# NREL/sup3r

Measured on AMD Instinct MI355X. Metric: samples/sec (lo-res chunks), generator forward, 5x/12x ST-GAN, higher is better.
Workload: dtype bf16

## Files before the change

### sup3r_amd/csrc/common.h

```cpp
#pragma once
#include <hip/hip_runtime.h>
#include <stdint.h>

#include <atomic>
#include <mutex>
#include <string>
#include <vector>

#include "../../include/sup3r_hip.h"
#include "launch_shape.h"


#define S3_OPTION_LIST(X) \
  X(BF16_TRAIN_ACT) \
  X(DENSE_WGS) \
  X(DGRAD_S2_MIN_TILES) \
  X(DISC_BF16) \
  X(FEWCH_HALO_MIN_TILES) \
  X(FP32_ACT) \
  X(GCONV_MF2) \
  X(GCONV_MF4) \
  X(GRAPH) \
  X(HALO32_MIN_TILES) \
  X(HALO_S2_MIN_TILES) \
  X(MFMA_DBG) \
  X(MFMA_TILE) \
  X(NO_BATCHED_PACK) \
  X(NO_BIAS_FUSE) \
  X(NO_CHUNKED_DY16) \
  X(NO_DGRAD_C2) \
  X(NO_DGRAD_C2_SLIDE) \
  X(DGRAD_C2_SLIDE_MIN_UNITS) \
  X(NO_DGRAD_CHUNKED) \
  X(NO_DGRAD_FEWCH) \
  X(NO_DGRAD_S2) \
  X(NO_DGRAD_X3) \
  X(NO_DIRECT_OUTPUT) \
  X(NO_DISC_BF16) \
  X(NO_DPRE16) \
  X(NO_DPRE16_ONLY_MASK) \
  X(NO_FEWCH) \
  X(NO_FEWCH_HALO) \
  X(NO_FEWPOS) \
  X(NO_FEWPOS_MFMA) \
  X(NO_FEWPOS_BWD_FUSE) \
  X(NO_FEWPOS_SMALL) \
  X(NO_FEWPOS_TRUNK) \
  X(NO_FOLD16) \
  X(NO_FRAME16) \
  X(NO_FUSED2D) \
  X(NO_GCONV) \
  X(NO_GCONV_DY16) \
  X(NO_GCONV_SPLITK) \
  X(NO_HALO32) \
  X(NO_HALO_S2) \
  X(NO_MASK_FUSE) \
  X(NO_MFMA_GEN) \
  X(NO_DGRAD_GEN) \
  X(NO_CONV2D_WS) \
  X(NO_TRAIN2D_BF16) \
  X(NO_ADD16) \
  X(NO_WS_EXO) \
  X(NO_WS_RES2) \
  X(NO_WS_PP) \
  X(NO_WS_X3) \
  X(WS_X3_MIN_POS) \
  X(NO_CONV2D_OUT) \
  X(NO_CONV2D_HEAD) \
  X(KEEP_ACTIVATIONS) \
  X(NO_MFMA_BWD) \
  X(NO_PERSIST) \
  X(NO_PERSIST_DGRAD) \
  X(NO_PERSIST_STRIP) \
  X(PERSIST2) \
  X(NO_REPEAT_FUSE) \
  X(NO_WGRAD_X3) \
  X(NO_GCONV_X3) \
  X(NO_SIGN_BYTES) \
  X(NO_HALO_S2_K64) \
  X(NO_PLAIN_FOLD16) \
  X(NO_SEG_REDUCE) \
  X(NO_TAIL_BAND) \
  X(NO_TAIL_MFMA) \
  X(NO_TAIL_SLIDE) \
  X(NO_TAIL_SWEEP) \
  X(NO_TAIL_WINDOW) \
  X(NO_TAIL_X3) \
  X(NO_TILE66) \
  X(NO_TILE_NF2) \
  X(NO_WGRAD_BF16) \
  X(NO_WGRAD_C2) \
  X(NO_WGRAD_GEN_PF) \
  X(NO_WGRAD_TAIL) \
  X(NO_WGRAD_TAIL_SWEEP) \
  X(NO_WGRAD_WS) \
  X(PERSIST_DGRAD_MIN_TILES) \
  X(PERSIST_MIN_TILES) \
  X(POISON_ALLOC) \
  X(TAIL_SWEEP_SHAPE) \
  X(TRACE) \
  X(WGRAD_DBG) \
  X(WGRAD_SIDE_STREAM)
enum S3OptId {
#define X(n) S3O_##n,
  S3_OPTION_LIST(X)
#undef X
  S3O_COUNT
};
struct S3Options {
  int32_t v[S3O_COUNT];
  bool has[S3O_COUNT];
  S3Options() { for (int i = 0; i < S3O_COUNT; ++i) { v[i] = 0; has[i] = false; } }
};
extern thread_local const S3Options* s3_active_options;
const char* s3_option_name(int id);
int s3_option_id(const char* name);
inline bool s3_opt_has(int id) { return s3_active_options && s3_active_options->has[id]; }
inline long long s3_opt_int(int id, long long dflt) { return s3_opt_has(id) ? s3_active_options->v[id] : dflt; }
inline bool s3_opt_on(int id) { return s3_opt_int(id, 0) != 0; }
struct S3OptScope {
  const S3Options* prev;
  explicit S3OptScope(const S3Options* o) : prev(s3_active_options) { s3_active_options = o; }
  ~S3OptScope() { s3_active_options = prev; }
};

struct s3_ctx {
// ... 28 lines not shown
  std::mutex m;
  bool done(int dev) const { return (mask.load(std::memory_order_acquire) >> (dev & 63)) & 1u; }
  void mark(int dev) { mask.fetch_or(1ull << (dev & 63), std::memory_order_release); }
};

#define S3_HIP(ctx, call)                                                    \
  do {                                                                       \
    hipError_t e_ = (call);                                                  \
    if (e_ != hipSuccess) {                                                  \
      (ctx)->err = std::string(#call) + ": " + hipGetErrorString(e_);        \
      return S3_EHIP;                                                        \
    }                                                                        \
  } while (0)

#define S3_FAIL(ctx, code, msg) \
  do {                          \
    (ctx)->err = (msg);         \
    return (code);              \
  } while (0)

inline int s3_lds_set(s3_ctx*) { return S3_OK; }
template <class K, class B, class... Rest>
int s3_lds_set(s3_ctx* ctx, K* kernel, B bytes, Rest... rest) {
  S3_HIP(ctx, hipFuncSetAttribute(reinterpret_cast<const void*>(kernel),
                                  hipFuncAttributeMaxDynamicSharedMemorySize, (int)bytes));
  return s3_lds_set(ctx, rest...);
}
template <class... Pairs>
inline int s3_lds_optin(s3_ctx* ctx, S3DeviceOnce& once, Pairs... pairs) {
  if (once.done(ctx->device)) return S3_OK;
  std::lock_guard<std::mutex> lk(once.m);
  const int rc = s3_lds_set(ctx, pairs...);
  if (rc == S3_OK) once.mark(ctx->device);
  return rc;
}

struct ConvGeom {
  int N;
  int D[3];
  int O[3];
  int Cin, Cout;
  int k[3], s[3], lo[3];
  int pad_mode;
  int act;
  float alpha;
  int d2s;
  int in_cstride = 0, in_cvalid = 0;
  int w_cin = 0;
  const float* exo = nullptr;
  const void* res2 = nullptr;
  int ws_only = 0;
  int in_rep = 0;
  int res_rep = 0;
  int gen = 0;
  int64_t xn = 0, yn = 0;
  int64_t xs[3] = {0, 0, 0}, ys[3] = {0, 0, 0}, yb[2] = {0, 0};
};

struct GatherGeom {
  int kind;
  int N;
  int Di[3], Ci;
  int Do[3], Co;
  int lo[3];
  int pad_mode;
  int rep;
  int d2s;
  int c_off;
};

__host__ __device__ inline int s3_reflect(int i, int n) {
  if (i < 0) i = -i;
  if (i > n - 1) i = 2 * (n - 1) - i;
  return i;
}

struct FastDiv {
  uint32_t d = 1, m = 1, sh1 = 0, sh2 = 0;
  FastDiv() = default;
  explicit FastDiv(uint32_t div) : d(div) {
    uint32_t l = 0;
    while (l < 32 && ((uint64_t)1 << l) < div) ++l;
    m = (uint32_t)((((uint64_t)1 << 32) * (((uint64_t)1 << l) - div)) / div + 1);
    sh1 = l < 1 ? l : 1;
    sh2 = l < 1 ? 0 : l - 1;
  }
  __device__ __forceinline__ uint32_t operator()(uint32_t x) const {
    const uint32_t t = __umulhi(m, x);
    return (t + ((x - t) >> sh1)) >> sh2;
  }
};

__device__ inline int s3_xcd_tile(int b, int nblk) {
  const int q = nblk / 8, r = nblk % 8, xcd = b % 8, k = b / 8;
  return (xcd < r ? xcd * (q + 1) : r * (q + 1) + (xcd - r) * q) + k;
}

__device__ inline void s3_xcd_share(int64_t n, int64_t& lo, int64_t& hi, int& k, int& nk) {
  const int G = gridDim.x, b = blockIdx.x, xcd = b % 8;
  int before = 0;
  for (int q = 0; q < xcd; ++q) before += (G - q + 7) / 8;
  nk = (G - xcd + 7) / 8;
  k = b / 8;
  lo = n * before / G;
  hi = n * (before + nk) / G;
}
// ... 298 lines not shown
```

### sup3r_amd/csrc/kernels_conv_mfma_persist.hip

```cpp
#include <cstdlib>

#include "wave_prims.h"

namespace {

constexpr int TS0 = 4, TS1 = 8, TS2 = 16;
constexpr int H0 = TS0 + 2, H1 = TS1 + 2, H2 = TS2 + 2;
constexpr int HP = H0 * H1 * H2;
constexpr int HALO_BYTES = HP * 128;
constexpr int SLAB_OFF = HALO_BYTES;
constexpr int BIAS_OFF = SLAB_OFF + 3 * 8192;
constexpr int LDS_BYTES = BIAS_OFF + 256;

constexpr int NCW = 8;
constexpr int NPW = 4;
constexpr int NTHR = (NCW + NPW) * 64;
constexpr int MFW = TS0 * TS1 / NCW;
constexpr int PT = NPW * 64;
constexpr int ROWC = H1 * H2;
constexpr int JR = (ROWC * 8 + PT - 1) / PT;
constexpr int NLATE = (H0 - 2) * JR;
static_assert(MFW * NCW == TS0 * TS1 && TS1 % MFW == 0 && MFW == 4, "tile / wave split");
static_assert(JR <= 6 && NLATE <= 24, "producer tap schedule");

constexpr int early_k(int t) { return (t >= 0 && t < JR) || (t >= 9 && t < 9 + JR) ? 1 : 0; }
constexpr int late_k(int t) { return t >= 0 && t < NLATE ? 1 : 0; }
constexpr int halo_k(int t) { return early_k(t) + late_k(t); }

template <int TW>
struct PGeo {
  static constexpr int TS1 = TW, H1 = TW + 2;
  static constexpr int HP = H0 * H1 * H2, HALO_BYTES = HP * 128, SLAB_OFF = HALO_BYTES;
  static constexpr int BIAS_OFF = SLAB_OFF + 3 * 8192, LDS_BYTES = BIAS_OFF + 256;
  static constexpr int MFW = TS0 * TW / NCW;
  static constexpr int ROWC = H1 * H2;
  static constexpr int JR = (ROWC * 8 + PT - 1) / PT;
  static constexpr int NLATE = (H0 - 2) * JR;
  static_assert(MFW * NCW == TS0 * TW && TW % MFW == 0 && (MFW == 4 || MFW == 3), "tile / wave split");
  static_assert(JR <= 6 && NLATE <= 24 && H0 + H1 + H2 <= 64, "producer tap schedule / halo table");
  static constexpr int early_k(int t) { return (t >= 0 && t < JR) || (t >= 9 && t < 9 + JR) ? 1 : 0; }
  static constexpr int late_k(int t) { return t >= 0 && t < NLATE ? 1 : 0; }
  static constexpr int halo_k(int t) { return early_k(t) + late_k(t); }
};

__device__ inline u32x4 ld16_async(const void* sbase, unsigned voff) {
  u32x4 v;
  asm volatile("global_load_dwordx4 %0, %1, %2" : "=v"(v) : "v"(voff), "s"(sbase) : "memory");
  return v;
}
__device__ inline void wait_vm_n(int n) {
  switch (n) {
    case 0: WAIT_VM(0); break;
    case 1: WAIT_VM(1); break;
    case 2: WAIT_VM(2); break;
    case 3: WAIT_VM(3); break;
    case 4: WAIT_VM(4); break;
    case 5: WAIT_VM(5); break;
    default: WAIT_VM(6); break;
  }
}

__global__ void pack_persist_kernel(const float* __restrict__ w,
                                    unsigned short* __restrict__ out, int cout, int n_ct) {
  const int total = n_ct * 27 * 64 * 64;
  for (int idx = blockIdx.x * blockDim.x + threadIdx.x; idx < total;
       idx += gridDim.x * blockDim.x) {
    const int ci = idx & 63, rho = (idx >> 6) & 63, tap = (idx >> 12) % 27, ct = (idx >> 12) / 27;
    const int co = ct * 64 + slab_row_cout(rho);
    const float v = co < cout ? w[((size_t)tap * 64 + ci) * cout + co] : 0.f;
    const unsigned u = pk2(v, 0.f);
    const int slot = (ci >> 3) ^ ((rho >> 1) & 7);
    out[(((size_t)ct * 27 + tap) * 64 + rho) * 64 + slot * 8 + (ci & 7)] = (unsigned short)(u & 0xFFFFu);
  }
}

__global__ void pack_jobs_kernel(const S3PackJob* __restrict__ jobs) {
  const S3PackJob jb = jobs[blockIdx.y];
  const int total = jb.n_ct * 27 * 64 * 64;
  for (int idx = blockIdx.x * blockDim.x + threadIdx.x; idx < total; idx += gridDim.x * blockDim.x) {
    const int ci = idx & 63, row = (idx >> 6) & 63, tap = (idx >> 12) % 27, ct = (idx >> 12) / 27;
    const int co = ct * 64 + row;
    float v = 0.f;
    if (co < jb.cout)
      v = jb.dgrad ? jb.w[((size_t)(26 - tap) * jb.cout + co) * 64 + ci]
                   : jb.w[((size_t)tap * 64 + ci) * jb.cout + co];
    const unsigned short h = (unsigned short)(pk2(v, 0.f) & 0xFFFFu);
    const size_t base = (((size_t)ct * 27 + tap) * 64) * 64;
    const int sw = (ci >> 3);
    jb.tile[base + (size_t)row * 64 + ((sw ^ ((row >> 1) & 7)) << 3) + (ci & 7)] = h;
    if (jb.persist) {
      const int nf = ((row >> 5) << 1) | ((row >> 2) & 1), kq = (row >> 3) & 3, r = row & 3;
      const int rho = nf * 16 + kq * 4 + r;
      jb.persist[base + (size_t)rho * 64 + ((sw ^ ((rho >> 1) & 7)) << 3) + (ci & 7)] = h;
    }
  }
}

template <int NFV, bool DG, int REP = 0, bool RIN = false, bool F16 = false, int TW = 8>
__global__ __launch_bounds__(NTHR) void conv3_mfma_persist_kernel(
    const unsigned short* __restrict__ x, const char* __restrict__ wimg,
    const float* __restrict__ bias, const unsigned short* __restrict__ res,
    unsigned short* __restrict__ y, ConvGeom g, int tiles0, int tiles1,
    int tiles2, int n_tiles, int ct, int gs0, int gs1) {
  using PG = PGeo<TW>;
  constexpr int TS1 = PG::TS1, H1 = PG::H1, HP = PG::HP, SLAB_OFF = PG::SLAB_OFF, BIAS_OFF = PG::BIAS_OFF;
  constexpr int MFW = PG::MFW, ROWC = PG::ROWC, JR = PG::JR, NLATE = PG::NLATE;
  (void)HP;
  extern __shared__ __attribute__((aligned(16))) char smem[];
  const int tid = threadIdx.x;
  const int lane = tid & 63;
  const int wave = __builtin_amdgcn_readfirstlane(tid >> 6);
  const int D0 = g.D[0], D1 = g.D[1], D2 = g.D[2];

  int h_cur, h_end;
  {
    const int nblk = gridDim.x, b = blockIdx.x;
    const int xcd = b % 8, k = b / 8;
    int rank = k;
    for (int xx = 0; xx < xcd; ++xx) rank += (nblk - xx + 7) / 8;
    const long long H = n_tiles;
    h_cur = (int)((rank * H) / nblk);
    h_end = (int)(((rank + 1) * H) / nblk);
  }
  auto tile_org = [&](int h, int& n, int& o0, int& o1, int& o2) __attribute__((always_inline)) {
    int tr = h;
    o0 = (tr % tiles0) * 2; tr /= tiles0;
    o2 = (tr % tiles2) * TS2; tr /= tiles2;
    o1 = (tr % tiles1) * TS1 + (DG ? 0 : gs1); tr /= tiles1;
    n = tr;
  };
  auto item_at = [&](int h, int& hs0, int& nr) __attribute__((always_inline)) {
    const bool whole = hs0 + 1 < tiles0 && h + 1 < h_end;
    nr = whole ? 4 : 2;
    hs0 += whole ? 2 : 1;
    if (hs0 >= tiles0) hs0 = 0;
    return h + (whole ? 2 : 1);
  };

  if (wave >= NCW) {
    const int pt = tid - NCW * 64;
    const int pw = wave - NCW;
    const unsigned dma_voff = (unsigned)(pw * 2048 + lane * 16);
    auto dma_slab = [&](int tap, int slot) __attribute__((always_inline)) {
      unsigned vo;
      asm volatile("v_mov_b32 %0, %1" : "=v"(vo) : "v"(dma_voff));
      const char* sb = wimg + (size_t)tap * 8192 + vo;
      char* d = smem + SLAB_OFF + slot * 8192 + __builtin_amdgcn_readfirstlane((int)vo);
      __builtin_amdgcn_global_load_lds(
          (const __attribute__((address_space(1))) void*)sb,
          (__attribute__((address_space(3))) void*)d, 16, 0, 0);
      __builtin_amdgcn_global_load_lds(
          (const __attribute__((address_space(1))) void*)(sb + 1024),
          (__attribute__((address_space(3))) void*)(d + 1024), 16, 0, 0);
    };
    const int pcell = pt >> 3, pch = pt & 7;
    const bool cdead = DG && g.in_cstride && pch * 8 >= g.in_cvalid;
    u32x4 hlate[NLATE], hrow[JR];
    unsigned in_off[JR];
    unsigned lds_off[JR];
    int htab = 0;
    const unsigned short* hx = x;
#pragma unroll
    for (int j = 0; j < JR; ++j) {
      int cell = pcell + 32 * j;
      if (cell > ROWC - 1) cell = ROWC - 1;
      lds_off[j] = (unsigned)(cell * 128 + ((pch ^ ((cell % H2) & 7)) << 4));
    }
#define HALO_TABLE(tile_expr)                                                          \
    {                                                                                  \
      int n_, o0_, o1_, o2_;                                                           \
      tile_org((tile_expr), n_, o0_, o1_, o2_);                                        \
      n_ = __builtin_amdgcn_readfirstlane(n_);                                         \
      const int ax = lane < H0 ? 0 : (lane < H0 + H1 ? 1 : 2);                         \
      const int c = lane - (ax == 0 ? 0 : (ax == 1 ? H0 : H0 + H1));                   \
      const int org = ax == 0 ? o0_ : (ax == 1 ? o1_ : o2_);                           \
         \
      constexpr bool rp = REP > 1 && RIN && !DG;                                       \
         \
         \
                                             \
      const int is2 = rp ? (ax >> 1) : 0;                         \
      const int D = (ax == 0 ? D0 : (ax == 1 ? D1 : D2)) * (1 + (REP > 1 ? REP - 1 : 0) * is2); \
      const int cs = (DG && g.in_cstride) ? g.in_cstride : 64;   \
      const int stride = ax == 0 ? D1 * D2 * cs : (ax == 1 ? D2 * cs : cs);            \
      if (DG) {                                                                        \
          \
            \
        const int E = D + 2, gsx = ax == 0 ? gs0 : (ax == 1 ? gs1 : 1);                \
        const int R = org + c - 1;                                                     \
// ... 10 lines not shown
      i = i < 0 ? 0 : (i > D - 1 ? D - 1 : i);                                         \
      if (rp) {                                                                        \
        if (REP == 2) i >>= is2;                                                       \
        else if (REP == 4) i >>= 2 * is2;                                              \
        else {    \
                       \
          const unsigned u = (unsigned)i;                                              \
          unsigned t = u + (u << 2);                                                   \
          t += t << 4;                                                                 \
          t += t << 8;                                                                 \
          i = (int)(u + (unsigned)is2 * (((t + u) >> 16) - u));                        \
        }                                                                              \
      }                                                                                \
      htab = i * stride;                                                               \
      hx = x + (size_t)n_ * D0 * D1 * D2 * 64;                                         \
      }                                                                                \
      _Pragma("unroll") for (int j = 0; j < JR; ++j) {                                 \
        int cell = pcell + 32 * j;                                                     \
        if (cell > ROWC - 1) cell = ROWC - 1;                                          \
        const int c1 = cell / H2, c2 = cell - c1 * H2;                                 \
        in_off[j] = (unsigned)__builtin_amdgcn_ds_bpermute((H0 + c1) << 2, htab) +     \
                    (unsigned)__builtin_amdgcn_ds_bpermute((H0 + H1 + c2) << 2, htab) + \
                    (cdead ? 0 : pch * 8);                                             \
      }                                                                                \
    }
    auto halo_load = [&](int r, int j) __attribute__((always_inline)) {
      const unsigned row = (unsigned)__builtin_amdgcn_readlane(htab, r);
      const unsigned eo = DG ? ((row + in_off[j]) & 0x3FFFFFFFu) : row + in_off[j];
      return ld16_async(hx, eo * 2);
    };
    auto halo_put = [&](int r, int j, const u32x4& v) __attribute__((always_inline)) {
      if (pcell + 32 * j < ROWC) {
        u32x4 w = v;
        if (DG) {
          asm volatile("" : "+v"(w));
          const unsigned row = (unsigned)__builtin_amdgcn_readlane(htab, r);
          if (((row + in_off[j]) >> 30) || cdead) w = (u32x4){0u, 0u, 0u, 0u};
        }
        unsigned lo = lds_off[j];
        if constexpr (REP > 1) {
          int cell = pcell + 32 * j;
          if (cell > ROWC - 1) cell = ROWC - 1;
          lo = (unsigned)(cell * 128 + ((pch ^ ((cell % H2) & 7)) << 4));
        }
        *reinterpret_cast<u32x4*>(smem + r * (ROWC * 128) + lo) = w;
      }
    };

    if (pt < 64)
      reinterpret_cast<float*>(smem + BIAS_OFF)[pt] =
          (bias && ct * 64 + slab_row_cout(pt) < g.Cout) ? bias[ct * 64 + slab_row_cout(pt)] : 0.f;
    dma_slab(0, 0);
    dma_slab(1, 1);
    if (h_cur < h_end) {
      HALO_TABLE(h_cur);
#pragma unroll
      for (int r = 0; r < H0; ++r) {
#pragma unroll
        for (int j = 0; j < JR; ++j) hrow[j] = halo_load(r, j);
        WAIT_VM(0);
#pragma unroll
        for (int j = 0; j < JR; ++j) halo_put(r, j, hrow[j]);
      }
    }
    WAIT_VM(0);
    WAIT_LGKM0();
    WG_BARRIER();

    for (int h = h_cur; h < h_end;) {
      int nr_, hs0_ = h % tiles0;
      h = item_at(h, hs0_, nr_);
#define has_next (h < h_end)
      HALO_TABLE(h < h_end - 1 ? h : h_end - 1);
#pragma unroll
      for (int tap = 0; tap < 27; ++tap) {
        if ((tap == 9 || tap == 18) && has_next) {
#pragma unroll
          for (int j = 0; j < JR; ++j) halo_put(tap == 9 ? 0 : 1, j, hrow[j]);
        }
        dma_slab((tap + 2) % 27, (tap + 2) % 3);
        if (tap < JR) hrow[tap % JR] = halo_load(0, tap % JR);
        if (tap >= 9 && tap < 9 + JR) hrow[(tap - 9) % JR] = halo_load(1, (tap - 9) % JR);
        if (tap < NLATE) hlate[tap % NLATE] = halo_load(2 + (tap % NLATE) / JR, (tap % NLATE) % JR);
        wait_vm_n(2 + PG::halo_k(tap) + PG::halo_k(tap - 1));
        WG_BARRIER();
      }
      if (has_next) {
#pragma unroll
        for (int u = 0; u < NLATE; ++u) halo_put(2 + u / JR, u % JR, hlate[u]);
      }
      WAIT_LGKM0();
      WG_BARRIER();
#undef has_next
    }
#undef HALO_TABLE
    return;
  }

  const int frow = lane & 15, kq = lane >> 4;
  const int mf0 = wave * MFW;
  const int row0 = (mf0 / TS1) * H1 + (mf0 % TS1);
  unsigned a_addr[3][2], b_addr[4][2];
#pragma unroll
  for (int c = 0; c < 3; ++c) {
    const int sw = (frow + c) & 7;
#pragma unroll
    for (int ks = 0; ks < 2; ++ks)
      a_addr[c][ks] = (unsigned)((row0 * H2 + frow + c) * 128 + (((ks * 4 + kq) ^ sw) << 4));
  }
#pragma unroll
  for (int nf = 0; nf < 4; ++nf) {
    const int rho = nf * 16 + frow;
#pragma unroll
    for (int ks = 0; ks < 2; ++ks)
      b_addr[nf][ks] = (unsigned)(SLAB_OFF + rho * 128 + (((ks * 4 + kq) ^ ((rho >> 1) & 7)) << 4));
  }
  const float slope = g.act == S3_ACT_LEAKY ? g.alpha : (g.act == S3_ACT_RELU ? 0.f : 1.f);
  const int db = REP > 1 ? 1 : g.d2s, cpo = REP > 1 ? g.Cout : g.Cout / (db * db);
  unsigned c_off[2];
  bool c_ok[2];
#pragma unroll
  for (int h = 0; h < 2; ++h) {
    const int co = ct * 64 + h * 32 + kq * 8;
    c_ok[h] = co < g.Cout;
    const int blk = co / cpo;
    c_off[h] = (unsigned)((((blk / db) * (g.O[1] * db) + blk % db) * g.O[2]) * cpo + co % cpo);
  }
  WG_BARRIER();
  __builtin_amdgcn_s_setprio(2);

  const int my_row = mf0 / TS1;
  for (int h = h_cur; h < h_end;) {
    int nr, n, org0, org1, org2;
    const int tile = h;
    tile_org(tile, n, org0, org1, org2);
    {
      int hs0 = org0 >> 1;
      h = item_at(h, hs0, nr);
    }
    if (my_row >= nr) {
#pragma unroll 1
      for (int t = 0; t < 28; ++t) WG_BARRIER();
      continue;
    }
    f32x4 acc[MFW][NFV];
#pragma unroll
    for (int nf = 0; nf < NFV; ++nf) {
      const f32x4 bv = *reinterpret_cast<const f32x4*>(smem + BIAS_OFF + (nf * 16 + kq * 4) * 4);
#pragma unroll
      for (int m = 0; m < MFW; ++m) acc[m][nf] = bv;
    }

    bf16x8 apre[MFW];
#pragma unroll
    for (int m = 0; m < MFW; ++m)
      apre[m] = *reinterpret_cast<const bf16x8*>(smem + a_addr[0][0] + (m * H2) * 128);
#pragma unroll 1
    for (int ta = 0; ta < 3; ++ta) {
      const unsigned ta_off = (unsigned)(ta * H1 * H2 * 128);
#pragma unroll
      for (int tb = 0; tb < 3; ++tb) {
#pragma unroll
        for (int tc = 0; tc < 3; ++tc) {
          bf16x8 bfr[NFV];
#pragma unroll
          for (int nf = 0; nf < NFV; ++nf)
            bfr[nf] = *reinterpret_cast<const bf16x8*>(smem + b_addr[nf][0] + tc * 8192);
#pragma unroll
          for (int m = 0; m < MFW; ++m)
#pragma unroll
            for (int nf = 0; nf < NFV; ++nf)
              acc[m][nf] = __builtin_amdgcn_mfma_f32_16x16x32_bf16(bfr[nf], apre[m], acc[m][nf], 0, 0, 0);
#pragma unroll
          for (int nf = 0; nf < NFV; ++nf)
            bfr[nf] = *reinterpret_cast<const bf16x8*>(smem + b_addr[nf][1] + tc * 8192);
#pragma unroll
          for (int m = 0; m < MFW; ++m) {
            const bf16x8 afr = *reinterpret_cast<const bf16x8*>(
                smem + a_addr[tc][1] + ta_off + ((m + tb) * H2) * 128);
#pragma unroll
            for (int nf = 0; nf < NFV; ++nf)
              acc[m][nf] = __builtin_amdgcn_mfma_f32_16x16x32_bf16(bfr[nf], afr, acc[m][nf], 0, 0, 0);
          }
          {
            const int ntc = tc < 2 ? tc + 1 : 0;
            const int ntb = tc < 2 ? tb : (tb < 2 ? tb + 1 : 0);
            const unsigned nta_off = (tc == 2 && tb == 2) ? ta_off + H1 * H2 * 128 : ta_off;
            if (!(tc == 2 && tb == 2) || ta < 2) {
#pragma unroll
              for (int m = 0; m < MFW; ++m)
                apre[m] = *reinterpret_cast<const bf16x8*>(
                    smem + a_addr[ntc][0] + nta_off + ((m + ntb) * H2) * 128);
// ... 52 lines not shown
    auto chunk_off = [&](int m, int h, bool& ok) __attribute__((always_inline)) {
      ok = c_ok[h] && e_ok[m] && 2 * h < NFV;
      return e_pos[m] + c_off[h];
    };
    uint4 rres[MFW][2];
    if (res) {
      const bool rr = REP > 1 && !DG && g.res_rep > 1;
      const int O2s = rr ? g.O[2] / (REP > 1 ? REP : 1) : g.O[2];
      const size_t r_base = rr ? (size_t)n * g.O[0] * g.O[1] * O2s * g.Cout : e_base;
#pragma unroll
      for (int m = 0; m < MFW; ++m) {
        unsigned r_pos = e_pos[m];
        if (rr) {
          const int mf = mf0 + m;
          const int o0 = org0 + mf / TS1, o1 = org1 + mf % TS1, o2 = org2 + frow;
          r_pos = (unsigned)(((o0 * g.O[1] + o1) * O2s + o2 / (REP > 1 ? REP : 1)) * cpo);
        }
#pragma unroll
        for (int h = 0; h < 2; ++h) {
          bool ok;
          chunk_off(m, h, ok);
          rres[m][h] = make_uint4(0, 0, 0, 0);
          if (ok) rres[m][h] = *reinterpret_cast<const uint4*>(res + r_base + r_pos + c_off[h]);
        }
      }
    }
#pragma unroll
    for (int m = 0; m < MFW; ++m) {
#pragma unroll
      for (int h = 0; h < 2; ++h) {
        bool ok;
        const unsigned off = chunk_off(m, h, ok);
        if (!ok) continue;
        float v[8];
#pragma unroll
        for (int q = 0; q < 8; ++q) {
          const float a = acc[m][(2 * h + (q >> 2)) % NFV][q & 3];
          const float sa = slope * a;
          asm("v_max_f32 %0, %1, %2" : "=v"(v[q]) : "v"(a), "v"(sa));
        }
        if (res) {
          const uint4 r = rres[m][h];
          v[0] += bf_lo(r.x); v[1] += bf_hi(r.x); v[2] += bf_lo(r.y); v[3] += bf_hi(r.y);
          v[4] += bf_lo(r.z); v[5] += bf_hi(r.z); v[6] += bf_lo(r.w); v[7] += bf_hi(r.w);
        }
        uint4 o;
        o.x = pk2(v[0], v[1]); o.y = pk2(v[2], v[3]);
        o.z = pk2(v[4], v[5]); o.w = pk2(v[6], v[7]);
        *reinterpret_cast<uint4*>(y + e_base + off) = o;
      }
    }
    WG_BARRIER();
  }
}

}

bool conv_mfma_persist_geom_ok(const ConvGeom& g) {
  if (g.Cin != 64 || g.Cout % 8 != 0 || g.Cout < 64 || g.d2s < 1) return false;
  if (g.D[2] < 8) return false;
  if (g.d2s > 1 && (g.Cout % (g.d2s * g.d2s) != 0 || (g.Cout / (g.d2s * g.d2s)) % 8 != 0))
    return false;
  if (g.pad_mode != S3_PAD_REFLECT) return false;
  if (g.act == S3_ACT_LEAKY && !(g.alpha >= 0.f && g.alpha <= 1.f)) return false;
  for (int d = 0; d < 3; ++d)
    if (g.k[d] != 3 || g.s[d] != 1) return false;
  return (int64_t)g.D[0] * g.D[1] * g.D[2] * 64 < (int64_t)1 << 31 &&
         (int64_t)g.O[0] * g.O[1] * g.O[2] * g.Cout < (int64_t)1 << 31;
}

bool conv_mfma_persist_dgrad_geom_ok(const ConvGeom& g) {
  if (g.Cin != 64 || (g.Cout != 64 && g.Cout != 32) || g.d2s != 1 || g.pad_mode != S3_PAD_ZERO ||
      g.act != S3_ACT_NONE)
    return false;
  for (int d = 0; d < 3; ++d)
    if (g.k[d] != 3 || g.s[d] != 1 || g.lo[d] != 2 || g.O[d] != g.D[d] + 2) return false;
  if (g.D[2] < 8) return false;
  if (g.in_cstride && ((g.in_cstride & 7) || (g.in_cvalid & 7) || g.in_cvalid < 8 || g.in_cvalid > 64)) return false;
  return (int64_t)g.N * g.D[0] * g.D[1] * g.D[2] * (g.in_cstride ? g.in_cstride : 64) < (int64_t)1 << 28;
}

static void persist_dgrad_grid(const ConvGeom& g, int* gs0, int* gs1) {
  int64_t best = -1;
  for (int a = 1; a <= g.N; ++a) {
    if (g.N % a) continue;
    const int b = g.N / a;
    const int64_t t = (int64_t)((a * g.O[0] + 1) / 2) * ((b * g.O[1] + TS1 - 1) / TS1);
    if (best < 0 || t < best) { best = t; *gs0 = a; *gs1 = b; }
  }
}

bool conv_mfma_persist_dgrad_supported(const s3_ctx* ctx, const ConvGeom& g) {
  if (s3_opt_on(S3O_NO_PERSIST_DGRAD)) return false;
  if (!conv_mfma_persist_dgrad_geom_ok(g)) return false;
  int gs0 = 1, gs1 = 1;
  persist_dgrad_grid(g, &gs0, &gs1);
  const int64_t halves = (int64_t)((gs0 * g.O[0] + 1) / 2) * ((gs1 * g.O[1] + TS1 - 1) / TS1) *
                         ((g.O[2] + TS2 - 1) / TS2);
  const int64_t tiles = (int64_t)((gs0 * g.O[0] + TS0 - 1) / TS0) * ((gs1 * g.O[1] + TS1 - 1) / TS1) *
                        ((g.O[2] + TS2 - 1) / TS2);
  const int64_t covered = halves * 2 * TS1 * TS2;
  const int64_t six = (int64_t)g.N * ((g.O[0] + 5) / 6) * ((g.O[1] + 5) / 6) * ((g.O[2] + 15) / 16) * 576;
  const int64_t min_tiles = s3_opt_has(S3O_PERSIST_DGRAD_MIN_TILES)
                                ? s3_opt_int(S3O_PERSIST_DGRAD_MIN_TILES, 0) : ctx->num_cu;
  return tiles >= min_tiles && covered * 10 <= six * 11;
}

int launch_conv_mfma_persist_dgrad(s3_ctx* ctx, const ConvGeom& g, const void* dpre16, const void* image,
                                   float* dxp, int accumulate, int frame16) {
  static S3DeviceOnce attr_set;
  if (int rc = s3_lds_optin(ctx, attr_set,
                            conv3_mfma_persist_kernel<4, true>, LDS_BYTES,
                            conv3_mfma_persist_kernel<2, true>, LDS_BYTES,
                            conv3_mfma_persist_kernel<4, true, 0, false, true>, LDS_BYTES)) return rc;
  if (frame16 && (accumulate || g.Cout != 64))
    S3_FAIL(ctx, S3_ESTATE, "persistent data gradient: a bf16 frame is written once, 64 channels wide");
  int gs0 = 1, gs1 = 1;
  persist_dgrad_grid(g, &gs0, &gs1);
  const int tiles0 = (gs0 * g.O[0] + 1) / 2, tiles1 = (gs1 * g.O[1] + TS1 - 1) / TS1,
            tiles2 = (g.O[2] + TS2 - 1) / TS2;
  const int n_tiles = tiles0 * tiles1 * tiles2;
  const int grid = persistent_grid(ctx->num_cu, (n_tiles + 1) / 2);
  auto kern = g.Cout <= 32 ? conv3_mfma_persist_kernel<2, true> : conv3_mfma_persist_kernel<4, true>;
  if (frame16) kern = conv3_mfma_persist_kernel<4, true, 0, false, true>;
  hipLaunchKernelGGL(kern, dim3(grid), dim3(NTHR), LDS_BYTES, ctx->stream,
                     (const unsigned short*)dpre16, (const char*)image, (const float*)nullptr,
                     (const unsigned short*)(accumulate ? dxp : nullptr), (unsigned short*)dxp, g, tiles0, tiles1,
                     tiles2, n_tiles, 0, gs0, gs1);
  S3_HIP(ctx, hipGetLastError());
  ++ctx->stat[S3_STAT_PERSIST_DGRAD];
  return S3_OK;
}

bool conv_mfma_persist_rep_ok(int rep) { return rep == 2 || rep == 3 || rep == 4; }

bool conv_mfma_persist_supported(const s3_ctx* ctx, const ConvGeom& g, ConvIO io,
                                 bool has_res) {
  if (s3_opt_on(S3O_NO_PERSIST)) return false;
  if (!io.in_bf16 || !io.out_bf16 || (has_res && !io.res_bf16)) return false;
  if (!conv_mfma_persist_geom_ok(g)) return false;
  if (has_res && g.d2s != 1) return false;
  const int64_t tiles = (int64_t)g.N * ((g.O[0] + TS0 - 1) / TS0) *
                        ((g.O[1] + TS1 - 1) / TS1) * ((g.O[2] + TS2 - 1) / TS2);
  return tiles >= s3_opt_int(S3O_PERSIST_MIN_TILES, ctx->num_cu * 7 / 16);
}

int launch_pack_jobs(s3_ctx* ctx, const S3PackJob* jobs_dev, int n_jobs, int max_ct) {
  if (n_jobs <= 0) return S3_OK;
  hipLaunchKernelGGL(pack_jobs_kernel, dim3(108 * max_ct, n_jobs), dim3(256), 0, ctx->stream, jobs_dev);
  S3_HIP(ctx, hipGetLastError());
  return S3_OK;
}

size_t conv_mfma_persist_image_bytes(const ConvGeom& g) {
  return (size_t)((g.Cout + 63) / 64) * 27 * 64 * 64 * 2;
}

int launch_conv_mfma_persist_pack(s3_ctx* ctx, const ConvGeom& g, const float* w, void* image) {
  const int n_ct = (g.Cout + 63) / 64;
  hipLaunchKernelGGL(pack_persist_kernel, dim3(108 * n_ct), dim3(256), 0, ctx->stream,
                     w, (unsigned short*)image, g.Cout, n_ct);
  S3_HIP(ctx, hipGetLastError());
  return S3_OK;
}

int launch_conv_mfma_persist(s3_ctx* ctx, const ConvGeom& g, const void* x,
                             const void* image, const float* bias,
                             const void* res, void* y) {
  static S3DeviceOnce attr_set;
#define S3_REP_ATTR(R)                                                                \
  conv3_mfma_persist_kernel<4, false, R, true>, LDS_BYTES,                            \
  conv3_mfma_persist_kernel<4, false, R, false>, LDS_BYTES,                           \
  conv3_mfma_persist_kernel<4, false, R, true, false, 6>, PGeo<6>::LDS_BYTES,         \
  conv3_mfma_persist_kernel<4, false, R, false, false, 6>, PGeo<6>::LDS_BYTES
  if (int rc = s3_lds_optin(ctx, attr_set,
                            conv3_mfma_persist_kernel<4, false>, LDS_BYTES,
                            conv3_mfma_persist_kernel<2, false>, LDS_BYTES,
                            S3_REP_ATTR(2), S3_REP_ATTR(3), S3_REP_ATTR(4),
                            conv3_mfma_persist_kernel<4, false, 0, false, false, 6>, PGeo<6>::LDS_BYTES,
                            conv3_mfma_persist_kernel<2, false, 0, false, false, 6>, PGeo<6>::LDS_BYTES)) return rc;
#undef S3_REP_ATTR
  const int tiles0 = (g.O[0] + 1) / 2, tiles1 = (g.O[1] + TS1 - 1) / TS1,
            tiles2 = (g.O[2] + TS2 - 1) / TS2;
  const int n_tiles = g.N * tiles0 * tiles1 * tiles2;
  const int grid = persistent_grid(ctx->num_cu, (n_tiles + 1) / 2);
  const int n_ct = (g.Cout + 63) / 64;
  const int rep = g.in_rep > 1 ? g.in_rep : (g.res_rep > 1 ? g.res_rep : 0);
  const bool rin = g.in_rep > 1;
  ConvGeom gk = g;
  if (rep) {
    bool ok = conv_mfma_persist_rep_ok(rep) && g.Cout == 64 && g.d2s == 1 &&
              !(g.in_rep > 1 && g.res_rep > 1 && g.in_rep != g.res_rep);
    for (int d = 0; d < 3; ++d) ok = ok && g.lo[d] == g.lo[0] && g.O[d] == g.D[d];
    if (!ok) S3_FAIL(ctx, S3_ESTATE, "persistent conv: unsupported fused temporal repeat");
    if (rin) gk.D[2] = g.D[2] / rep;
  }
  const int rem1 = g.O[1] % TS1;
  const int64_t strip_halves = (int64_t)g.N * tiles0 * tiles2;
  if (rem1 >= 1 && rem1 <= 6 && g.O[1] > TS1 && strip_halves >= 2 * (int64_t)ctx->num_cu &&
      (!rep || n_ct == 1) && !s3_opt_on(S3O_NO_PERSIST_STRIP)) {
    const int t1a = g.O[1] / TS1;
    const int na = g.N * tiles0 * t1a * tiles2, nb = (int)strip_halves;
    const int ga = persistent_grid(ctx->num_cu, (na + 1) / 2), gb = persistent_grid(ctx->num_cu, (nb + 1) / 2);
    for (int ct = 0; ct < n_ct; ++ct) {
      const bool half = g.Cout - ct * 64 <= 32;
      const char* img = (const char*)image + (size_t)ct * 27 * 8192;
      auto k8 = half ? conv3_mfma_persist_kernel<2, false> : conv3_mfma_persist_kernel<4, false>;
      auto k6 = half ? conv3_mfma_persist_kernel<2, false, 0, false, false, 6>
                     : conv3_mfma_persist_kernel<4, false, 0, false, false, 6>;
      if (rep == 2) {
        k8 = rin ? conv3_mfma_persist_kernel<4, false, 2, true> : conv3_mfma_persist_kernel<4, false, 2, false>;
        k6 = rin ? conv3_mfma_persist_kernel<4, false, 2, true, false, 6>
                 : conv3_mfma_persist_kernel<4, false, 2, false, false, 6>;
      } else if (rep == 3) {
        k8 = rin ? conv3_mfma_persist_kernel<4, false, 3, true> : conv3_mfma_persist_kernel<4, false, 3, false>;
        k6 = rin ? conv3_mfma_persist_kernel<4, false, 3, true, false, 6>
                 : conv3_mfma_persist_kernel<4, false, 3, false, false, 6>;
      } else if (rep == 4) {
        k8 = rin ? conv3_mfma_persist_kernel<4, false, 4, true> : conv3_mfma_persist_kernel<4, false, 4, false>;
        k6 = rin ? conv3_mfma_persist_kernel<4, false, 4, true, false, 6>
                 : conv3_mfma_persist_kernel<4, false, 4, false, false, 6>;
      }
      hipLaunchKernelGGL(k8, dim3(ga), dim3(NTHR), LDS_BYTES, ctx->stream, (const unsigned short*)x, img, bias,
                         (const unsigned short*)res, (unsigned short*)y, gk, tiles0, t1a, tiles2, na, ct, 1, 0);
      hipLaunchKernelGGL(k6, dim3(gb), dim3(NTHR), PGeo<6>::LDS_BYTES, ctx->stream, (const unsigned short*)x,
                         img, bias, (const unsigned short*)res, (unsigned short*)y, gk, tiles0, 1, tiles2, nb,
                         ct, 1, t1a * TS1);
    }
    S3_HIP(ctx, hipGetLastError());
    return S3_OK;
  }
  for (int ct = 0; ct < n_ct; ++ct) {
    const bool half = g.Cout - ct * 64 <= 32;
    auto kern = half ? conv3_mfma_persist_kernel<2, false> : conv3_mfma_persist_kernel<4, false>;
    if (rep == 2) kern = rin ? conv3_mfma_persist_kernel<4, false, 2, true> : conv3_mfma_persist_kernel<4, false, 2, false>;
    else if (rep == 3) kern = rin ? conv3_mfma_persist_kernel<4, false, 3, true> : conv3_mfma_persist_kernel<4, false, 3, false>;
    else if (rep == 4) kern = rin ? conv3_mfma_persist_kernel<4, false, 4, true> : conv3_mfma_persist_kernel<4, false, 4, false>;
    hipLaunchKernelGGL(kern, dim3(grid), dim3(NTHR), LDS_BYTES, ctx->stream,
                       (const unsigned short*)x, (const char*)image + (size_t)ct * 27 * 8192, bias,
                       (const unsigned short*)res, (unsigned short*)y, gk, tiles0,
                       tiles1, tiles2, n_tiles, ct, 1, 0);
  }
  S3_HIP(ctx, hipGetLastError());
  return S3_OK;
}
```

### sup3r_amd/csrc/plan.cpp

```cpp
#include <algorithm>
#include <cstdio>
#include <cstring>

#include "plan_internal.h"

int plan_alloc(s3_plan* pl, void** out, size_t bytes) {
  s3_ctx* ctx = pl->ctx;
  if (bytes == 0) bytes = 16;
  S3_HIP(ctx, hipMalloc(out, bytes));
  S3_HIP(ctx, hipMemsetAsync(*out, s3_opt_has(S3O_POISON_ALLOC) ? 0xFF : 0, bytes, ctx->stream));
  pl->owned.push_back(*out);
  pl->total_bytes += bytes;
  return S3_OK;
}

static int64_t numel5(const int64_t* d) { return d[0] * d[1] * d[2] * d[3] * d[4]; }

static void fill_conv_geom(const s3_plan* pl, const s3_op_desc& d, ConvGeom& g) {
  const TensorRec& in = pl->t[d.in0];
  const TensorRec& out = pl->t[d.out];
  g.N = (int)in.dims[0];
  for (int i = 0; i < 3; ++i) {
    g.D[i] = (int)in.dims[1 + i];
    g.k[i] = d.k[i]; g.s[i] = d.stride[i]; g.lo[i] = d.lo[i];
// ... 343 lines not shown
              const bool gc_out16 = disc16 && o.gconv() && d.res < 0 && o.cg.Cout % 8 == 0 &&
                                    (o.cg.Cin == 2 || o.cg.Cin == 4 || (deep16 && o.cg.Cin % 8 == 0));
              if (!tail16 && !gc_in16) demote(d.in0, changed);
              demote(d.res, changed);
              if (!gc_out16) demote(d.out, changed);
            } else {
              const bool small = d.res < 0 && !o.fewpos() &&
                                 (conv_small_supported(o.cg, 1) || conv_tail_mfma_supported(o.cg));
              if (!small) demote(d.in0, changed);
              demote(d.res, changed);
              if (small || o.fewpos()) demote(d.out, changed);
            }
            break;
          case S3_OP_REPEAT_T: case S3_OP_D2S: case S3_OP_PAD: case S3_OP_CROP:
          case S3_OP_ROLL_T: case S3_OP_DILATE:
            if (dt[root_of(pl, d.in0)] != dt[root_of(pl, d.out)]) {
              demote(d.in0, changed);
              demote(d.out, changed);
            }
            break;
          case S3_OP_VIEW:
            break;
          case S3_OP_ADD:
            if (training || d.bcast_c || (pl->t[d.out].numel & 7) || s3_opt_has(S3O_NO_ADD16) ||
                !(dt[root_of(pl, d.in0)] && dt[root_of(pl, d.in1)] && dt[root_of(pl, d.out)])) {
              demote(d.in0, changed); demote(d.in1, changed); demote(d.out, changed);
            }
            break;
          default:
            demote(d.in0, changed); demote(d.in1, changed);
            demote(d.res, changed); demote(d.out, changed);
            break;
        }
      }
    }
    for (int i = 0; i < n_tensors; ++i) pl->t[i].dtype = dt[root_of(pl, i)];
  }
  for (auto& o : pl->ops) {
    if (o.d.kind != S3_OP_CONV) continue;
    o.io.in_bf16 = pl->t[root_of(pl, o.d.in0)].dtype;
    o.io.out_bf16 = pl->t[root_of(pl, o.d.out)].dtype;
    o.io.res_bf16 = o.d.res >= 0 ? pl->t[root_of(pl, o.d.res)].dtype : 0;
  }
}

static void plan_ws_only(s3_plan* pl) {
  const int precision = pl->precision;
  for (auto& o : pl->ops)
    if (o.d.kind == S3_OP_CONV && o.fam == Fam::MFMA && conv_mfma_is_gen(o.cg, precision) && o.cg.in_rep <= 1 &&
        conv2d_ws_supported(o.cg, precision, o.io, o.d.res >= 0))
      o.cg.ws_only = 1;
}

static bool plan_ws_split_holds(const s3_plan* pl) {
  const int precision = pl->precision;
  for (auto& o : pl->ops) {
    if (o.d.kind != S3_OP_CONV || (o.exo_src < 0 && o.res2_src < 0)) continue;
    if (conv2d_ws_supported(o.cg, precision, o.io, o.d.res >= 0) &&
        (o.res2_src < 0 || pl->t[root_of(pl, o.res2_src)].dtype == 1))
      continue;
    return false;
  }
  return true;
}

static void plan_mask_fusion(s3_plan* pl) {
  const int training = pl->training, output = pl->output;
  const int n_ops = (int)pl->ops.size(), n_tensors = (int)pl->t.size();
  if (!training) return;
  std::vector<int> ncons(n_tensors, 0), prod(n_tensors, -1);
  for (int i = 0; i < n_ops; ++i) {
    const s3_op_desc& d = pl->ops[i].d;
    for (int id : {d.in0, d.in1, d.res})
      if (id >= 0) ++ncons[root_of(pl, id)];
    if (d.kind != S3_OP_VIEW) prod[root_of(pl, d.out)] = i;
  }
  for (auto& o : pl->ops) {
    if (o.d.kind == S3_OP_CONV) {
      const int pr = prod[root_of(pl, o.d.in0)];
      if (pr >= 0 && pl->ops[pr].d.kind == S3_OP_CONV) o.in_prod = pr;
    }
    const bool fold = (dgrad_is_mfma(o.dgrad) && !dgrad_is_valid(o.dgrad)) ||
                      (o.dgrad == Dgrad::FEWPOS_MFMA && o.cg.pad_mode == S3_PAD_REFLECT);
    if (o.d.kind != S3_OP_CONV || !(dgrad_is_s2(o.dgrad) || fold)) continue;
    const int r = root_of(pl, o.d.in0);
    const int pi = prod[r];
    if (pi < 0 || ncons[r] != 1 || r == root_of(pl, output) || pl->t[r].is_input) continue;

    if (fold && (o.cg.Cin & 3)) continue;
    const OpRec& po = pl->ops[pi];
    if (po.d.kind == S3_OP_CONV && po.cg.act != S3_ACT_NONE && po.cg.d2s == 1 && po.d.res < 0)
      o.mask_prod = pi;
  }
}

static void plan_repeat_fusion(s3_plan* pl) {
  s3_ctx* ctx = pl->ctx;
  const int precision = pl->precision, training = pl->training, output = pl->output;
  const int n_ops = (int)pl->ops.size();
  if (training || precision != S3_PREC_BF16 || s3_opt_has(S3O_NO_REPEAT_FUSE)) return;
  for (int i = 0; i < n_ops; ++i) {
    OpRec& r = pl->ops[i];
    if (r.d.kind != S3_OP_REPEAT_T || !conv_mfma_persist_rep_ok(r.d.rep)) continue;
    const int rt = root_of(pl, r.d.out);
    if (rt == root_of(pl, output) || pl->t[root_of(pl, r.d.in0)].dtype != pl->t[rt].dtype) continue;
    bool ok = true;
// ... 235 lines not shown
            w == Wgrad::BF16_TRUNK || w == Wgrad::F32_TRUNK, dgrad_is_mfma(d), dgrad_is_c2(d), dgrad_is_s2(d),
            d == Dgrad::GCONV);
  }
}

extern "C" int s3_plan_create_opt(s3_ctx* ctx, s3_params* params,
                                  const s3_tensor_desc* tensors, int n_tensors,
                                  const s3_op_desc* ops, int n_ops,
                                  const int32_t* inputs, int n_inputs,
                                  int32_t output, int precision, int training,
                                  const s3_plan_options* options, s3_plan** out) {
  if (!ctx || !params || !tensors || !ops || !out) return S3_EINVAL;
  if (output < 0 || output >= n_tensors) S3_FAIL(ctx, S3_EINVAL, "plan: bad output id");
  S3Options plan_opt = ctx->opt;
  if (int orc = apply_options(ctx, plan_opt, options)) return orc;
  s3_plan* pl = new s3_plan();
  pl->opt = plan_opt;
  S3OptScope opt_scope(&pl->opt);
  pl->ctx = ctx; pl->params = params; pl->precision = precision;
  pl->training = training; pl->output = output;
  pl->t.resize(n_tensors);
  for (int i = 0; i < n_tensors; ++i) {
    memcpy(pl->t[i].dims, tensors[i].dims, sizeof(int64_t) * 5);
    pl->t[i].numel = numel5(tensors[i].dims);
    if (pl->t[i].numel <= 0) { delete pl; S3_FAIL(ctx, S3_EINVAL, "plan: empty tensor"); }
  }
  for (int i = 0; i < n_inputs; ++i) {
    if (inputs[i] < 0 || inputs[i] >= n_tensors) { delete pl; S3_FAIL(ctx, S3_EINVAL, "plan: bad input id"); }
    pl->inputs.push_back(inputs[i]);
    pl->t[inputs[i]].is_input = true;
  }
  pl->ops.resize(n_ops);
  WorkspaceSizes ws;
  if (int rc = plan_select(pl, ops, ws)) { delete pl; return rc; }
  plan_ws_exo(pl);
  plan_ws_res2(pl);
  plan_dtypes(pl);
  plan_trace(pl);
  plan_ws_only(pl);
  if (!plan_ws_split_holds(pl)) {
    delete pl;
    ++tl_no_ws_exo;
    const int rc = s3_plan_create_opt(ctx, params, tensors, n_tensors, ops, n_ops, inputs, n_inputs, output,
                                      precision, training, options, out);
    --tl_no_ws_exo;
    return rc;
  }

  plan_mask_fusion(pl);
  plan_dpre16(pl, ws);
  plan_repeat_fusion(pl);
  for (auto& o : pl->ops)
    if (o.d.kind == S3_OP_CONV) o.fwd = resolve_fwd(ctx, o, precision);
  size_t max_t = 0;
  int rc = plan_arena(pl, max_t);
  if (!rc) rc = plan_workspace(pl, ws, max_t);
  if (rc) { s3_plan_destroy(pl); return rc; }
  plan_fused2d(pl);
  *out = pl;
  return S3_OK;
}

void graph_drop(s3_plan* pl) {
  if (pl->graph_exec) (void)hipGraphExecDestroy(pl->graph_exec);
  if (pl->graph) (void)hipGraphDestroy(pl->graph);
  pl->graph_exec = nullptr;
  pl->graph = nullptr;
}

extern "C" void s3_plan_destroy(s3_plan* pl) {
  if (!pl) return;
  (void)hipStreamSynchronize(pl->ctx->stream);
  graph_drop(pl);
  if (pl->cap_stream) (void)hipStreamDestroy(pl->cap_stream);
  for (auto& e : pl->prof_ev) (void)hipEventDestroy(e);
  for (void* p : pl->owned) (void)hipFree(p);
  fused2d_free(pl->fused2d);
  delete pl;
}
```

Before: 2006.

## Interleave persistent conv tile walk across XCD blocks with alternating direction

```diff
diff --git a/sup3r_amd/csrc/common.h b/sup3r_amd/csrc/common.h
--- a/sup3r_amd/csrc/common.h
+++ b/sup3r_amd/csrc/common.h
@@ -72,6 +72,10 @@
   X(NO_PERSIST) \
   X(NO_PERSIST_DGRAD) \
   X(NO_PERSIST_STRIP) \
+  X(NO_XCD_WALK) \
+  X(XCD_WALK_CHUNK) \
+  X(XCD_WALK_CONTIG) \
+  X(XCD_WALK_REV) \
   X(PERSIST2) \
   X(NO_REPEAT_FUSE) \
   X(NO_WGRAD_X3) \
@@ -206,6 +210,7 @@
   int ws_only = 0;
   int in_rep = 0;
   int res_rep = 0;
+  int xcd_walk = 0;
   int gen = 0;
   int64_t xn = 0, yn = 0;
   int64_t xs[3] = {0, 0, 0}, ys[3] = {0, 0, 0}, yb[2] = {0, 0};
diff --git a/sup3r_amd/csrc/kernels_conv_mfma_persist.hip b/sup3r_amd/csrc/kernels_conv_mfma_persist.hip
--- a/sup3r_amd/csrc/kernels_conv_mfma_persist.hip
+++ b/sup3r_amd/csrc/kernels_conv_mfma_persist.hip
@@ -1,3 +1,4 @@
+#include <algorithm>
 #include <cstdlib>
 
 #include "wave_prims.h"
@@ -101,7 +102,7 @@
     const unsigned short* __restrict__ x, const char* __restrict__ wimg,
     const float* __restrict__ bias, const unsigned short* __restrict__ res,
     unsigned short* __restrict__ y, ConvGeom g, int tiles0, int tiles1,
-    int tiles2, int n_tiles, int ct, int gs0, int gs1) {
+    int tiles2, int n_tiles, int ct, int gs0, int gs1, int walk) {
   using PG = PGeo<TW>;
   constexpr int TS1 = PG::TS1, H1 = PG::H1, HP = PG::HP, SLAB_OFF = PG::SLAB_OFF, BIAS_OFF = PG::BIAS_OFF;
   constexpr int MFW = PG::MFW, ROWC = PG::ROWC, JR = PG::JR, NLATE = PG::NLATE;
@@ -112,16 +113,39 @@
   const int wave = __builtin_amdgcn_readfirstlane(tid >> 6);
   const int D0 = g.D[0], D1 = g.D[1], D2 = g.D[2];
 
-  int h_cur, h_end;
+  int h_cur, h_end, wk;
   {
     const int nblk = gridDim.x, b = blockIdx.x;
     const int xcd = b % 8, k = b / 8;
-    int rank = k;
-    for (int xx = 0; xx < xcd; ++xx) rank += (nblk - xx + 7) / 8;
+    int before = 0;
+    for (int xx = 0; xx < xcd; ++xx) before += (nblk - xx + 7) / 8;
     const long long H = n_tiles;
-    h_cur = (int)((rank * H) / nblk);
-    h_end = (int)(((rank + 1) * H) / nblk);
-  }
+    if (!walk) {
+      const int rank = before + k;
+      h_cur = (int)((rank * H) / nblk);
+      h_end = (int)(((rank + 1) * H) / nblk);
+      wk = 32 + 30;
+    } else {
+      const bool contig = (walk & 64) != 0;
+      const int cs = walk & 31, nk = contig ? 1 : (nblk - xcd + 7) / 8;
+      const int kk = contig ? 0 : k, first = contig ? before + k : before;
+      const int cpc = ((tiles0 - 1) >> cs) + 1;
+      const long long Q = (long long)(n_tiles / tiles0) * cpc;
+      const int qlo = (int)(Q * first / nblk), qhi = (int)(Q * (first + nk) / nblk);
+      const int mine = qhi - qlo > kk ? (qhi - qlo - kk + nk - 1) / nk : 0;
+      auto h_of = [&](int q) { const int c = q / cpc; return c * tiles0 + (q - c * cpc) * (1 << cs); };
+      const bool rev = (walk & 32) != 0;
+      h_cur = h_of(rev ? qlo + kk + (mine - 1) * nk : qlo + kk);
+      h_end = h_of(rev ? qlo : qhi);
+      wk = (rev ? -nk : nk) * 32 + cs;
+    }
+  }
+  auto wk_now = [&]() __attribute__((always_inline)) {
+    int w = wk;
+    asm volatile("" : "+s"(w));
+    return w;
+  };
+  auto in_walk = [&](int h) __attribute__((always_inline)) { return ((h - h_end) ^ (wk_now() >> 31)) < 0; };
   auto tile_org = [&](int h, int& n, int& o0, int& o1, int& o2) __attribute__((always_inline)) {
     int tr = h;
     o0 = (tr % tiles0) * 2; tr /= tiles0;
@@ -129,12 +153,18 @@
     o1 = (tr % tiles1) * TS1 + (DG ? 0 : gs1); tr /= tiles1;
     n = tr;
   };
-  auto item_at = [&](int h, int& hs0, int& nr) __attribute__((always_inline)) {
-    const bool whole = hs0 + 1 < tiles0 && h + 1 < h_end;
+  auto item_at = [&](int h, int col, int hs0, int& nr) __attribute__((always_inline)) {
+    const int w = wk_now(), cs = w & 31, r = hs0 >> cs;
+    int cend = (r + 1) << cs;
+    if (cend > tiles0) cend = tiles0;
+    const bool whole = hs0 + 1 < cend && in_walk(h + 1);
     nr = whole ? 4 : 2;
-    hs0 += whole ? 2 : 1;
-    if (hs0 >= tiles0) hs0 = 0;
-    return h + (whole ? 2 : 1);
+    const int st = whole ? 2 : 1;
+    if (hs0 + st < cend) return h + st;
+    const int cpc = ((tiles0 - 1) >> cs) + 1;
+    const int q = col * cpc + r + (w >> 5);
+    const int c = q / cpc;
+    return c * tiles0 + (q - c * cpc) * (1 << cs);
   };
 
   if (wave >= NCW) {
@@ -251,7 +281,7 @@
           (bias && ct * 64 + slab_row_cout(pt) < g.Cout) ? bias[ct * 64 + slab_row_cout(pt)] : 0.f;
     dma_slab(0, 0);
     dma_slab(1, 1);
-    if (h_cur < h_end) {
+    if (in_walk(h_cur)) {
       HALO_TABLE(h_cur);
 #pragma unroll
       for (int r = 0; r < H0; ++r) {
@@ -266,11 +296,12 @@
     WAIT_LGKM0();
     WG_BARRIER();
 
-    for (int h = h_cur; h < h_end;) {
-      int nr_, hs0_ = h % tiles0;
-      h = item_at(h, hs0_, nr_);
-#define has_next (h < h_end)
-      HALO_TABLE(h < h_end - 1 ? h : h_end - 1);
+    for (int h = h_cur; in_walk(h);) {
+      const int h0_ = h, col_ = h / tiles0;
+      int nr_;
+      h = item_at(h, col_, h - col_ * tiles0, nr_);
+#define has_next in_walk(h)
+      HALO_TABLE(has_next ? h : h0_);
 #pragma unroll
       for (int tap = 0; tap < 27; ++tap) {
         if ((tap == 9 || tap == 18) && has_next) {
@@ -329,14 +360,11 @@
   __builtin_amdgcn_s_setprio(2);
 
   const int my_row = mf0 / TS1;
-  for (int h = h_cur; h < h_end;) {
+  for (int h = h_cur; in_walk(h);) {
     int nr, n, org0, org1, org2;
     const int tile = h;
     tile_org(tile, n, org0, org1, org2);
-    {
-      int hs0 = org0 >> 1;
-      h = item_at(h, hs0, nr);
-    }
+    h = item_at(h, h / tiles0, org0 >> 1, nr);
     if (my_row >= nr) {
 #pragma unroll 1
       for (int t = 0; t < 28; ++t) WG_BARRIER();
@@ -495,6 +523,31 @@
     }
     WG_BARRIER();
   }
+}
+
+int persist_walk(int nh0, int H, int grid, int mode) {
+  if (s3_opt_on(S3O_NO_XCD_WALK) || grid < 1) return 0;
+  bool rev = mode == 2;
+  if (s3_opt_has(S3O_XCD_WALK_REV)) rev = s3_opt_on(S3O_XCD_WALK_REV);
+  const int dir = rev ? 32 : 0, contig = s3_opt_on(S3O_XCD_WALK_CONTIG) ? 64 : 0;
+  if (s3_opt_has(S3O_XCD_WALK_CHUNK)) {
+    const int n = (int)s3_opt_int(S3O_XCD_WALK_CHUNK, 2);
+    for (int l = 1; l < 16; ++l)
+      if (n == 1 << l) return l + dir + contig;
+    return 30 + dir;
+  }
+  if (!mode) return 0;
+  const int cs = 1;
+  const int64_t cpc = ((nh0 - 1) >> cs) + 1, Q = (int64_t)(H / nh0) * cpc;
+  int64_t worst = 0, before = 0;
+  for (int xcd = 0; xcd < 8 && xcd < grid; ++xcd) {
+    const int nk = (grid - xcd + 7) / 8;
+    const int64_t share = Q * (before + nk) / grid - Q * before / grid;
+    worst = std::max(worst, ((share + nk - 1) / nk) << cs);
+    before += nk;
+  }
+  if (worst <= ((int64_t)H + grid - 1) / grid) return cs + dir + contig;
+  return 0;
 }
 
 }
@@ -569,7 +622,7 @@
   hipLaunchKernelGGL(kern, dim3(grid), dim3(NTHR), LDS_BYTES, ctx->stream,
                      (const unsigned short*)dpre16, (const char*)image, (const float*)nullptr,
                      (const unsigned short*)(accumulate ? dxp : nullptr), (unsigned short*)dxp, g, tiles0, tiles1,
-                     tiles2, n_tiles, 0, gs0, gs1);
+                     tiles2, n_tiles, 0, gs0, gs1, persist_walk(tiles0, n_tiles, grid, 0));
   S3_HIP(ctx, hipGetLastError());
   ++ctx->stat[S3_STAT_PERSIST_DGRAD];
   return S3_OK;
@@ -665,10 +718,11 @@
                  : conv3_mfma_persist_kernel<4, false, 4, false, false, 6>;
       }
       hipLaunchKernelGGL(k8, dim3(ga), dim3(NTHR), LDS_BYTES, ctx->stream, (const unsigned short*)x, img, bias,
-                         (const unsigned short*)res, (unsigned short*)y, gk, tiles0, t1a, tiles2, na, ct, 1, 0);
+                         (const unsigned short*)res, (unsigned short*)y, gk, tiles0, t1a, tiles2, na, ct, 1, 0,
+                         persist_walk(tiles0, na, ga, 0));
       hipLaunchKernelGGL(k6, dim3(gb), dim3(NTHR), PGeo<6>::LDS_BYTES, ctx->stream, (const unsigned short*)x,
                          img, bias, (const unsigned short*)res, (unsigned short*)y, gk, tiles0, 1, tiles2, nb,
-                         ct, 1, t1a * TS1);
+                         ct, 1, t1a * TS1, persist_walk(tiles0, nb, gb, 0));
     }
     S3_HIP(ctx, hipGetLastError());
     return S3_OK;
@@ -682,7 +736,7 @@
     hipLaunchKernelGGL(kern, dim3(grid), dim3(NTHR), LDS_BYTES, ctx->stream,
                        (const unsigned short*)x, (const char*)image + (size_t)ct * 27 * 8192, bias,
                        (const unsigned short*)res, (unsigned short*)y, gk, tiles0,
-                       tiles1, tiles2, n_tiles, ct, 1, 0);
+                       tiles1, tiles2, n_tiles, ct, 1, 0, persist_walk(tiles0, n_tiles, grid, g.xcd_walk ? 1 + ((g.xcd_walk - 1 + ct) & 1) : 0));
   }
   S3_HIP(ctx, hipGetLastError());
   return S3_OK;
diff --git a/sup3r_amd/csrc/plan.cpp b/sup3r_amd/csrc/plan.cpp
--- a/sup3r_amd/csrc/plan.cpp
+++ b/sup3r_amd/csrc/plan.cpp
@@ -419,6 +419,13 @@
       o.cg.ws_only = 1;
 }
 
+static void plan_xcd_walk(s3_plan* pl) {
+  if (pl->training) return;
+  int n = 0;
+  for (auto& o : pl->ops)
+    if (o.d.kind == S3_OP_CONV && o.fwd == Fwd::MFMA_PERSIST) o.cg.xcd_walk = 1 + (n++ & 1);
+}
+
 static bool plan_ws_split_holds(const s3_plan* pl) {
   const int precision = pl->precision;
   for (auto& o : pl->ops) {
@@ -760,6 +767,7 @@
   plan_repeat_fusion(pl);
   for (auto& o : pl->ops)
     if (o.d.kind == S3_OP_CONV) o.fwd = resolve_fwd(ctx, o, precision);
+  plan_xcd_walk(pl);
   size_t max_t = 0;
   int rc = plan_arena(pl, max_t);
   if (!rc) rc = plan_workspace(pl, ws, max_t);
```

New measurement: 2018, median of 6. No clear change (+0.6%).
